# huggingface/tokenizers

Measured on AMD Instinct MI355X. Metric: GB input text/sec (whole node), GPT-2 BPE encode_batch, higher is better.
Workload: dtype u8->u32

## Files before the change

### tokenizers_amd/csrc/capi/pipeline.cpp

```cpp

int lookup_grid(const tkamd_tokenizer* t) { return std::min(3 * t->n_cu, (int)NSQ); }

struct QueueSizes {
    uint32_t sq_cap[4], row_base[4];
    size_t total;
};
static bool rerun_wanted(tkamd_tokenizer* t, Workspace* w, int raw) {
    const int err = raw & ~NOTE_BITS;
    bool again = false;
    if (raw & NOTE_ADDED_SEEN) { t->added_spec_pause = t->added_spec_len; w->force_general = true; again = true; }
    if (raw & NOTE_NFC_SEEN) { t->nfc_spec_pause = t->nfc_spec_len; w->force_nfc = true; ++t->nfc_reruns; again = true; }
    if (err == ERR_QUEUE_FULL && t->q16_div > 1) { t->q16_div = t->q16_div > 2 ? 2 : 1; again = true; }
    return again;
}

QueueSizes queue_sizes(size_t N, uint32_t q16_div, int grid) {
    QueueSizes z{};
    const size_t n_tiles = N / LOOKUP_TILE_BYTES + 1;
    const size_t per_sq = ((n_tiles + grid - 1) / grid) * LOOKUP_TILE_BYTES;
    z.sq_cap[0] = (uint32_t)(per_sq / q16_div + 64);
    z.sq_cap[1] = (uint32_t)(per_sq / 17 + 16);
    z.sq_cap[2] = (uint32_t)(per_sq / 33 + 16);
    z.sq_cap[3] = (uint32_t)(per_sq / 65 + 16);
    size_t acc = 0;
    for (int c = 0; c < 4; ++c) { z.row_base[c] = (uint32_t)acc; acc += (size_t)z.sq_cap[c] * (size_t)grid; }
    z.total = acc;
    return z;
}

void reserve_workspace(tkamd_tokenizer* t, Workspace* w, int64_t n_bytes, int64_t n_docs, uint32_t flags, bool want_meta) {
    int64_t W = (n_bytes >> 6) + 2;
    size_t N = (size_t)n_bytes;
    w->w_docmask.reserve(W * 8);
    w->w_startmask.reserve(W * 8);
    w->w_wprefix.reserve(W * 4);
    w->w_bsum.reserve((W / 256 + 2) * 4);
    w->w_tok0.reserve((N + 4) * 4);
    w->w_tmp_ids.reserve((N + 4) * 4);
    const QueueSizes z = queue_sizes(N, t->q16_div, lookup_grid(t));
    w->w_rows.reserve(z.total * 16);
    w->w_queues.reserve(z.total * 8);
    w->w_cstate.reserve((N / COMPACT_CHUNK + 4) * 8 + 16);
    w->w_chunk_lo.reserve((N / COMPACT_CHUNK + 4) * 4);
    w->w_qcount.reserve((size_t)QCNT_WORDS * 4);
    w->w_pt_tokoff.reserve((N + 4) * 4);
    w->w_ids.reserve((N + 4) * 4);
    w->w_doc_pt.reserve((n_docs + 2) * 4);
    w->w_tok_offsets.reserve((n_docs + 2) * 8);
    w->w_scalars.reserve(SC_SLOTS * 8);
    if (want_meta) w->w_pt_start.reserve((N + 4) * 4);
    if (flags & TKAMD_OFFSETS_MASK) {
        w->w_tmp_end.reserve((N + 4) * 4);
        w->w_offsets.reserve((N + 4) * 8);
    }
    if (flags & TKAMD_WANT_WORD_IDS) w->w_word_ids.reserve((N + 4) * 4);
}

using ull = unsigned long long;
enum class Step { Done, Again };

struct Batch {
    tkamd_tokenizer* t; Workspace* w; const uint8_t* d_text; const int64_t* d_doc_off; int64_t n_docs, n_bytes; const int64_t* d_seq_off; int64_t n_seqs;
    uint32_t flags; hipStream_t st; tkamd_device_result* out; const int64_t* d_inp_off; int64_t n_inputs;
    HostModel& hm = t->hm;
    Prof pf{t, w, st};
    bool mixed = false, want_words = false, want_meta = false, add_special = false, prefix_space = false, metaspace = false, words_in = false, pairs = false;
    bool typed_single = false, has_epilogue = false, want_overflow = false;
    bool precomp = false;
    int64_t n_p = 0;
    const uint8_t* p_text = nullptr; const int64_t *p_doc_off = nullptr, *d_plen = nullptr; const uint32_t* p_norig = nullptr;
    bool nfc_general = false;
    uint32_t off_mode = 0, mcap = 0;
    int64_t n_x = 0, e_n = 0, W0 = 0, W = 0;
    int64_t *sc = nullptr, *d_npretok = nullptr, *d_ntok_total = nullptr, *d_xlen = nullptr, *d_nseg = nullptr;
    uint32_t *d_counters = nullptr, *n_match = nullptr;
    int *d_err = nullptr, grid = 0;
    size_t claim_slots = 0;
    bool use_claims = false, lean = false;
    const int64_t *raw_doc_off = nullptr, *e_tok_off = nullptr;
    bool have_raw = false, have_norm = false, have_added = false;
    const ull* matchmask = nullptr;
    size_t seg_cap = 0, WX = 0;
    const uint8_t* x_text = nullptr;
    const int64_t *x_doc_off = nullptr, *x_len_dev = nullptr, *piece_off = nullptr, *piece_n_dev = nullptr;
    const uint32_t *norig = nullptr, *norig_e = nullptr;
    int64_t n_in = 0;
    bool lead_done = false;
    bool has_end = false;
    bool meta_masks = false;
    uint32_t *mlist = nullptr, *tmp_end = nullptr, *pt_end = nullptr;
    const uint32_t* pt_word = nullptr;
    WordCache wc{nullptr, nullptr, nullptr, 0u, nullptr};

    void check_request(); void zero_batch_state(); void validate_inputs(); void empty_batch();
    void build_x_text(); void pretokenize(); void run_model(); void compact_and_meta(); Step epilogue();
// ... 38 lines not shown
            while (p > 0 && !t->nfc_spec_pause.compare_exchange_weak(p, p - 1)) {}
            nfc_general = p > 0;
        }
    }
    precomp = hm.norm == NORM_PRECOMPILED;
    n_p = precomp ? (int64_t)hm.pc_growth * n_bytes + 64 : n_bytes;
    if (precomp && n_p >= (int64_t)0x55555500ll) throw Invalid("batch larger than 4 GiB behind the normalizer's bound: split it (byte offsets are 32-bit on the device)");
    n_x = (hm.norm == NORM_BERT || nfc_general) ? 3 * n_bytes + 64
          : metaspace ? 3 * n_p + 3 * (n_docs + 2 * (int64_t)mcap + 1) + 64
          : n_bytes + (prefix_space ? n_docs + (int64_t)mcap : 0);
    if (n_x >= (int64_t)0xFFFFFF00ll) throw Invalid("batch larger than 4 GiB: split it (byte offsets are 32-bit on the device)");
    const bool bpe_path = hm.model == MODEL_BPE && !hm.char_bpe && (hm.pretok == PT_BYTELEVEL_GPT2 || hm.pretok == PT_LLAMA3 || hm.pretok == PT_SPLIT_CHAIN || hm.pretok == PT_DIGITS_GPT2 ||
                                                                      hm.pretok == PT_BYTELEVEL_NOREGEX);
    const bool local_pretok = hm.pretok == PT_WHITESPACE || hm.pretok == PT_WHITESPACE_SPLIT || hm.pretok == PT_BERT;
    const bool word_models = (hm.model == MODEL_WORDLEVEL || hm.model == MODEL_WORDPIECE) && local_pretok;
    const bool char_bpe = hm.model == MODEL_BPE && hm.char_bpe && (local_pretok || metaspace);
    const bool unigram = hm.model == MODEL_UNIGRAM && metaspace;
    if (!bpe_path && !word_models && !char_bpe && !unigram)
        throw Unsupported("this build covers {ByteLevel(GPT-2 regex), Llama-3 Split+ByteLevel, ByteLevel(no regex)}+BPE and "
                          "{Whitespace,WhitespaceSplit,BertPreTokenizer}+{WordLevel,WordPiece,BPE over characters} and the U+2581 front+{BPE over characters, Unigram}");
    if (prefix_space && hm.norm != NORM_NONE) throw Unsupported("ByteLevel add_prefix_space behind a normalizer");
    words_in = n_seqs >= 0;
    if (words_in && !d_seq_off) throw Invalid("null sequence offsets");
    e_n = words_in ? n_seqs : n_docs;
    pairs = (flags & TKAMD_PAIRS) != 0 || mixed;
    if (pairs && !mixed && (e_n & 1)) throw Invalid("TKAMD_PAIRS: an odd number of documents");
    if (pairs && (flags & TKAMD_ADD_SPECIAL) && !hm.pp_pair_unsupported.empty()) throw Unsupported("add_special_tokens on a pair: " + hm.pp_pair_unsupported);
    typed_single = !pairs && hm.pp_single_typed;
    has_epilogue = hm.trunc_on || hm.pad_on || pairs || typed_single;
    want_overflow = (flags & TKAMD_WANT_OVERFLOW) != 0 && hm.trunc_on;
    W0 = (n_bytes >> 6) + 1;
    W = (n_x >> 6) + 1;
    grid = t->n_cu * 8;
}

void Batch::zero_batch_state() {
    reserve_workspace(t, w, (hm.norm == NORM_NFC && w->device_bound) ? 3 * n_bytes + 64 : n_x, n_docs, flags, want_meta);
    sc = w->w_scalars.as<int64_t>();
    d_npretok = sc + SC_NPRETOK;
    d_ntok_total = sc + SC_NTOK;
    d_xlen = sc + SC_NKEPT;
    d_err = (int*)(sc + SC_ERR);
    d_counters = (uint32_t*)(sc + SC_COUNTERS);
    const char* const claims_hook = test_hook("TKAMD_CLAIMS");
    const bool claims_on = !(claims_hook && !strcmp(claims_hook, "0"));
    use_claims = claims_on && !t->word_cache &&
                 (hm.model == MODEL_BPE || hm.model == MODEL_UNIGRAM || (hm.model == MODEL_WORDPIECE && hm.max_input_chars >= (uint32_t)WORD_MAX_KEY));
    if (use_claims) {
        int p = t->claims_pause.load();
        while (p > 0 && !t->claims_pause.compare_exchange_weak(p, p - 1)) {}
        if (p > 0) use_claims = false;
    }
    w->last_used_claims = use_claims;
    const size_t cstate_bytes = (((size_t)n_x / (size_t)COMPACT_CHUNK + 4) * 8 + 15) & ~(size_t)15;
    ZeroRegions z{};
    z.add(sc, SC_SLOTS * 8);
    if (!(hm.norm == NORM_BERT || metaspace)) z.add(w->w_docmask.p, (size_t)(W + 1) * 8);
    z.add(w->w_qcount.p, (size_t)QCNT_WORDS * 4);
    z.add(w->w_cstate.p, cstate_bytes);
    if (hm.pretok == PT_LLAMA3 && split_rule_fast(hm.split_rule)) {
        w->w_l3_tiles.reserve(l3_tileflag_words(n_x) * 8);
        z.add(w->w_l3_tiles.p, l3_tileflag_words(n_x) * 8);
    }
    if (use_claims) {
        constexpr size_t per_slot = 64;
        int bits = 18;
        while (bits < 24 && ((size_t)1 << bits) < (size_t)n_bytes / per_slot) ++bits;
        claim_slots = (size_t)1 << bits;
        w->w_claims.reserve(claim_slots * 16);
        w->w_claim_rows.reserve(claim_slots * 16);
        z.add(w->w_claims.p, claim_slots * 16);
    }
    launch_zero_regions(st, t->n_cu * 4, z);
    out->d_ids = w->w_ids.as<uint32_t>();
    out->d_tok_offsets = w->w_tok_offsets.as<int64_t>();
    out->d_n_tokens = d_ntok_total;
    out->d_n_pretokens = d_npretok;
    out->ids_capacity = ((hm.norm == NORM_NFC && w->device_bound) ? 3 * n_bytes + 64 : n_x) + 4;
    out->d_offsets = out->d_word_ids = out->d_pad_counts = out->d_enc_docs = out->d_enc_parts = nullptr;
    out->d_type_ids = out->d_seq_ids = nullptr;
    out->d_n_encodings = nullptr;
    w->cur_trim1 = nullptr;
    w->last_n_enc = -1;
    w->last_n_docs = n_docs;
    w->last_seq_off = d_seq_off;
    w->last_n_seqs = n_seqs;
    w->last_inp_off = d_inp_off;
    w->last_n_inputs = n_inputs;
}

void Batch::validate_inputs() {
    w->w_doc_off.reserve((size_t)(n_docs + 2) * 8);
    lean = n_bytes > 0 && hm.at[0].size() == 0 && hm.at[1].size() == 0 && (hm.norm == NORM_NONE || (hm.norm == NORM_NFC && !nfc_general)) && !prefix_space &&
           (hm.pretok == PT_BYTELEVEL_GPT2 || hm.pretok == PT_BYTELEVEL_NOREGEX);
    raw_doc_off = d_doc_off;
    if (!lean) {
        pf.begin("validate_csr");
        launch_validate_csr(st, d_doc_off, n_docs, n_bytes, d_err, w->w_doc_off.as<int64_t>());
        pf.end();
    }
    d_doc_off = w->w_doc_off.as<int64_t>();
    if (words_in) {
        w->w_seq_off.reserve((size_t)(n_seqs + 2) * 8);
        w->w_seq_tok_off.reserve((size_t)(n_seqs + 2) * 8);
        launch_validate_csr(st, d_seq_off, n_seqs, n_docs, d_err, w->w_seq_off.as<int64_t>());
        d_seq_off = w->w_seq_off.as<int64_t>();
        out->d_tok_offsets = w->w_seq_tok_off.as<int64_t>();
// ... 763 lines not shown
```

### tokenizers_amd/csrc/kernels.hpp

```cpp
#pragma once
#include <hip/hip_runtime_api.h>
#include <cstdint>

#include "nfc_core.hpp"
#include "precompiled_core.hpp"
#include "tables.hpp"

namespace tkamd {

struct DevTables {
    const uint16_t* uc1;
    const uint8_t* uc2;
    const uint32_t* byte_id;
    const MergeSlot* merges;
    const uint16_t* merge_disp;
    uint32_t merge_mask, merge_seed, merge_bmask;
    uint32_t newid_affine, newid_base;
    const uint32_t* char_id;
    uint32_t cb;
    int* err;
    uint32_t* probes;
    void* pub_rows;
    uint32_t* pub_pos;
    uint32_t pub_mask;
// ... 323 lines not shown
void launch_pair_lens(hipStream_t st, const PairArgs& a);
void launch_pair_overflow_scan(hipStream_t st, const PairArgs& a, int64_t* n_enc);
void launch_pair_ranges(hipStream_t st, const PairArgs& a);
void launch_pair_finalize(hipStream_t st, int grid, const PairArgs& a);
void launch_added_match(hipStream_t st, const AddedArgs& a, const uint8_t* text, int64_t n_bytes, const int64_t* len_dev, const int64_t* seg_off, int64_t n_segs,
                        const int64_t* n_segs_dev, const unsigned long long* skipmask, const uint16_t* uc1, const uint8_t* uc2, unsigned long long* candmask,
                        uint32_t* sents, uint32_t* n_sents, uint32_t* match_list, uint32_t* n_match, uint32_t cap, uint32_t len_flag, int* err);
void launch_added_detect(hipStream_t st, const AddedArgs& a, const uint8_t* text, int64_t n_bytes, const int64_t* len_dev, int* note);
void launch_scatter_matches(hipStream_t st, const uint32_t* list, const uint32_t* n_list, int64_t n_bytes, const int64_t* len_dev, unsigned long long* matchmask,
                            unsigned long long* spanmask, unsigned long long* stopmask, unsigned long long* hardmask, uint32_t* tmp_end, uint32_t* dirty);
void launch_mask_or2(hipStream_t st, unsigned long long* dst, const unsigned long long* a, const unsigned long long* b, int64_t n_words);
void launch_emit_boundaries(hipStream_t st, const unsigned long long* mask, const uint32_t* wprefix, int64_t n_bytes, const int64_t* len_dev, const int64_t* total, int64_t* out);
void launch_metaspace(hipStream_t st, const uint8_t* text, int64_t n_bytes, const int64_t* doc_off, int64_t n_docs, const unsigned long long* pstart,
                      const unsigned long long* dstart, const unsigned long long* mmask, const unsigned long long* smask, uint32_t prepend, uint8_t* olen,
                      uint32_t* wsum, uint32_t* bsum, uint32_t* wbase, int64_t* x_len, uint8_t* xtext, uint32_t* nos, int64_t* xdoc_off,
                      const int64_t* len_dev = nullptr, const uint32_t* map = nullptr);
void launch_precompiled(hipStream_t st, const PcTables& pt, const uint8_t* text, int64_t n_bytes, const int64_t* doc_off, int64_t n_docs, const unsigned long long* verbatim,
                        const unsigned long long* bound, uint8_t* olen, uint16_t* ltot, uint32_t* wsum, uint32_t* bsum, uint32_t* wbase, int64_t* x_len, uint8_t* ntext,
                        uint32_t* nos, int64_t* ndoc_off, int* err, int grid, int64_t out_cap);
void launch_pc_translate_matches(hipStream_t st, uint32_t* list, const uint32_t* n_list, const uint8_t* olen, const uint16_t* ltot, const uint32_t* wbase, int64_t n_bytes,
                                 const int64_t* x_len);
void launch_ms_units(hipStream_t st, const uint8_t* xtext, int64_t n_x, const int64_t* x_len, const unsigned long long* pmask, unsigned long long* startmask,
                     int64_t n_words, bool split);
void launch_ms_piece_rank(hipStream_t st, const unsigned long long* startmask, const uint32_t* wprefix, const unsigned long long* pmask, const uint32_t* pprefix,
                          int64_t n_x, const int64_t* x_len, uint32_t* pt_word);
void launch_translate_matches_norm(hipStream_t st, uint32_t* list, const uint32_t* n_list, const uint8_t* olen, const uint32_t* wbase, int64_t n_bytes, const int64_t* x_len);
void launch_translate_matches_prefix(hipStream_t st, uint32_t* list, const uint32_t* n_list, const unsigned long long* bmask, const uint32_t* wprefix, int64_t n_bytes,
                                     const int64_t* len_dev, const int64_t* total, const int64_t* xseg_off);
void launch_prefix_doc_csr(hipStream_t st, const int64_t* doc_off, int64_t n_docs, const unsigned long long* bmask, const uint32_t* wprefix, int64_t n_bytes,
                           const int64_t* len_dev, const int64_t* total, const int64_t* xseg_off, int64_t* xdoc_off);
void launch_mask_or(hipStream_t st, unsigned long long* dst, const unsigned long long* src, int64_t n_words, const uint32_t* n_list);
void launch_apply_matches(hipStream_t st, unsigned long long* startmask, unsigned long long* endmask, const unsigned long long* matchmask,
                          const unsigned long long* spanmask, const unsigned long long* stopmask, int64_t n_words, const uint32_t* n_list);
void launch_apply_match_ids(hipStream_t st, const uint32_t* match_list, const uint32_t* n_match, const unsigned long long* startmask,
                            const uint32_t* wprefix, uint32_t* tok0);
void launch_decode(hipStream_t st, const uint32_t* ids, const int64_t* tok_off, int64_t n_docs, int64_t n_tok, const void* entry, uint32_t n_ids,
                   const uint8_t* blob, uint32_t skip_special, uint32_t* firstmask, uint32_t* len, uint32_t* bsum, uint32_t* pos, int64_t* total,
                   int64_t* out_off, uint8_t* out_bytes_or_null, uint32_t from_end = 0, uint32_t* badmask = nullptr, uint32_t* dupmask = nullptr);
int prepare_long_kernel();
void launch_bpe_merge_long(hipStream_t st, int grid, const DevTables& t, const uint8_t* text, const QView& v, void* rows,
                           uint32_t* tmp_ids, uint32_t* tmp_end, uint32_t* list_huge, uint32_t* n_huge,
                           uint32_t* scratch, unsigned long long scratch_words, unsigned long long* scratch_used, int* err);
void launch_bpe_merge_long_only(hipStream_t st, int grid, const DevTables& t, const uint8_t* text, const QView& v, void* rows, uint32_t* tmp_ids, uint32_t* tmp_end,
                                uint32_t* list_huge, uint32_t* n_huge);
void launch_word_cache_insert(hipStream_t st, int grid, const DevTables& t, const uint8_t* text, const QView& v, const void* rows, const WordCache& wc);
void launch_compact(hipStream_t st, int grid, const uint32_t* tok0, const void* rows, const void* cache_rows, const uint32_t* tmp_ids, const int64_t* n_pretok,
                    unsigned long long* state, int64_t* n_tok, uint32_t* pt_tokoff, uint32_t* ids, const uint32_t* chunk_lo, const uint32_t* doc_pt,
                    int64_t n_docs, int64_t* tok_offsets, void* phases = nullptr, uint8_t* tok_b8 = nullptr);
int compact_grid(int n_cu);
void launch_zero_regions(hipStream_t st, int grid, const ZeroRegions& z);
void launch_zero_tail(hipStream_t st, uint8_t* p, const int64_t* len_dev, int n, unsigned long long* mask = nullptr, int64_t mask_words = 0, int grid = 1);
constexpr int CP_ITEMS_PER_LANE = 4;
constexpr int COMPACT_CHUNK = 256 * CP_ITEMS_PER_LANE;
const char* test_hook(const char* name);

}
```

### tokenizers_amd/csrc/kernels/output.hip

```cpp

constexpr int CP_NT = 256;
template <int CP_ITEMS> struct CpShape {
    static constexpr int CHUNK = CP_NT * CP_ITEMS;
    static constexpr int STAGE = CP_ITEMS * 640;
    static_assert(CP_ITEMS == 2 || CP_ITEMS == 4 || CP_ITEMS == 8, "shapes the launcher knows");
};

template <int CP_ITEMS> struct CpRows {
    uint4 row[CP_ITEMS];
    uint32_t cnt[CP_ITEMS];
};
template <int CP_ITEMS> struct CpTok0 { uint32_t w[CP_ITEMS]; };
template <int CP_ITEMS>
__device__ __forceinline__ void cp_load_tok0(const uint32_t* __restrict__ tok0, int64_t p0, int64_t P, CpTok0<CP_ITEMS>& f) {
    static_assert(CP_ITEMS == 2 || CP_ITEMS == 4 || CP_ITEMS == 8, "one 8-byte, one or two 16-byte loads of tok0 per lane");
    uint32_t* const first = f.w;
    const bool whole = p0 + CP_ITEMS <= P;
    const int64_t pl = whole ? p0 : 0;
    if (CP_ITEMS == 2) {
        const uint2 a = load_nt((const uint2*)(tok0 + pl));
        first[0] = a.x; first[CP_ITEMS - 1] = a.y;
    } else {
        const uint4 a = load_nt((const uint4*)(tok0 + pl));
        first[0] = a.x; first[1] = a.y; first[CP_ITEMS > 2 ? 2 : 0] = a.z; first[CP_ITEMS > 3 ? 3 : 0] = a.w;
// ... 30 lines not shown
    }
    return v;
}
template <int CP_ITEMS>
__device__ __forceinline__ uint32_t cp_load_rows(const CpTok0<CP_ITEMS>& f, const uint4* __restrict__ rows, const uint4* __restrict__ crows, CpRows<CP_ITEMS>& r) {
    CpGather<CP_ITEMS> g;
    cp_issue_rows<CP_ITEMS>(f, rows, crows, g);
    return cp_settle_rows<CP_ITEMS>(f, g, r);
}
template <int CP_ITEMS>
__device__ __forceinline__ uint32_t cp_load(const uint32_t* __restrict__ tok0, const uint4* __restrict__ rows, const uint4* __restrict__ crows, int64_t p0, int64_t P, CpRows<CP_ITEMS>& r) {
    CpTok0<CP_ITEMS> f;
    cp_load_tok0<CP_ITEMS>(tok0, p0, P, f);
    return cp_load_rows<CP_ITEMS>(f, rows, crows, r);
}
#define TKAMD_CP_SCATTER(DST, R, O, RAW, B8)                                                                  \
    _Pragma("unroll") for (int k = 0; k < CP_ITEMS; ++k) {                                                    \
        const uint32_t c = (R).cnt[k];                                                                        \
        if (c) {                                                                                              \
            const bool more = ((R).row[k].x >> ROW_CNT_SHIFT) == ROW_CNT_MORE;                                \
            const uint32_t keep_ = (RAW) ? 0xFFFFFFFFu : TOK_ID_MASK;                                         \
            (DST)[(O)] = ((R).row[k].x & ROW_ID_MASK) | ((RAW) && (B8) ? B8_FIRST << ROW_B8_SHIFT : 0u);      \
            if (!(RAW) && (B8)) (B8)[(O)] = (uint8_t)B8_FIRST;                                                \
            if (!more) {                                                                                      \
                if (c > 1) { (DST)[(O) + 1] = (R).row[k].y & keep_; if (!(RAW) && (B8)) (B8)[(O) + 1] = (uint8_t)((R).row[k].y >> ROW_B8_SHIFT); } \
                if (c > 2) { (DST)[(O) + 2] = (R).row[k].z & keep_; if (!(RAW) && (B8)) (B8)[(O) + 2] = (uint8_t)((R).row[k].z >> ROW_B8_SHIFT); } \
                if (c > 3) { (DST)[(O) + 3] = (R).row[k].w & keep_; if (!(RAW) && (B8)) (B8)[(O) + 3] = (uint8_t)((R).row[k].w >> ROW_B8_SHIFT); } \
            } else {                                                                                          \
                if (!(RAW) && (B8)) for (uint32_t j = 1; j < c; ++j) (B8)[(O) + j] = 0;                       \
                 \
                 \
                const uint32_t* const src_ = tmp_ids + (R).row[k].y;                                          \
                for (uint32_t j = 1; j < c; j += 4) {                                                         \
                    const Unaligned16 v_ = *(const Unaligned16*)(src_ + j);                                   \
                    (DST)[(O) + j] = v_.a;                                                                    \
                    if (j + 1 < c) (DST)[(O) + j + 1] = v_.b;                                                 \
                    if (j + 2 < c) (DST)[(O) + j + 2] = v_.c;                                                 \
                    if (j + 3 < c) (DST)[(O) + j + 3] = v_.d;                                                 \
                }                                                                                             \
            }                                                                                                 \
        }                                                                                                     \
        (O) += c;                                                                                             \
    }

template <int CP_ITEMS, bool PROF = false, bool EARLY = true>
__global__ __launch_bounds__(CP_NT, CP_ITEMS == 8 ? 2 : 5) void k_compact(const uint32_t* __restrict__ tok0, const uint4* __restrict__ rows, const uint4* __restrict__ crows,
                                                   const uint32_t* __restrict__ tmp_ids, const int64_t* __restrict__ n_pretok,
                                                   unsigned long long* __restrict__ state,
                                                   int64_t* __restrict__ n_tok, uint32_t* __restrict__ pt_tokoff, uint32_t* __restrict__ ids,
                                                   const uint32_t* __restrict__ chunk_lo, const uint32_t* __restrict__ doc_pt, int64_t n_docs,
                                                   int64_t* __restrict__ tok_offsets, unsigned long long* __restrict__ phases, uint32_t patience,
                                                   uint8_t* __restrict__ tok_b8) {
    constexpr int CP_CHUNK = CpShape<CP_ITEMS>::CHUNK, CP_STAGE = CpShape<CP_ITEMS>::STAGE;
    unsigned long long ph_t = 0ull, ph_t0 = 0ull, ph_acc[4] = {0ull, 0ull, 0ull, 0ull};
    auto tick = [&](int k) {
        if (PROF && threadIdx.x == 0) { const unsigned long long now = __builtin_amdgcn_s_memtime(); ph_acc[k] += now - ph_t; ph_t = now; }
    };
    if (PROF && threadIdx.x == 0) ph_t = ph_t0 = __builtin_amdgcn_s_memtime();
    __shared__ uint32_t sm[4];
    __shared__ uint32_t s_dlo[2], s_dhi[2];
    __shared__ uint32_t s_docpt[2][CP_NT];
    __shared__ uint32_t s_stage[2][CP_STAGE];
    __shared__ uint32_t s_loc[2][CP_CHUNK];
    __shared__ uint32_t s_tot[2];
    __shared__ unsigned long long s_lbw;
    const int64_t P = uniform_i64(*n_pretok);
    const int64_t n_chunks = (P + CP_CHUNK - 1) / CP_CHUNK;
    const int tid = (int)threadIdx.x;
    if (n_chunks == 0) {
        if (blockIdx.x == 0)
            for (int64_t d = tid; d <= n_docs; d += CP_NT) tok_offsets[d] = 0;
        return;
    }
    auto front = [&](int64_t ch, int b, const CpAhead<CP_ITEMS>& a) {
        const uint32_t dlo = a.dlo, dhi = a.dhi;
        CpRows<CP_ITEMS> r;
        const bool has_doc = dlo + (uint32_t)tid < dhi;
        uint32_t my_docpt = 0u;
        const uint32_t v = cp_load_rows<CP_ITEMS>(a.f, rows, crows, r);
        if (has_doc) my_docpt = doc_pt[dlo + (uint32_t)tid];
        uint32_t tot;
        const uint32_t ex = block256_excl_scan(v, sm, &tot);
        if (tid == 0) { lb_publish(state, ch, (unsigned long long)tot); s_tot[b] = tot; }
        if (has_doc) s_docpt[b][tid] = my_docpt;
        if (tid == 0) { s_dlo[b] = dlo; s_dhi[b] = dhi; }
        tick(0);
        uint32_t acc = ex;
#pragma unroll
        for (int k = 0; k < CP_ITEMS; ++k) { s_loc[b][tid * CP_ITEMS + k] = acc; acc += r.cnt[k]; }
        if (tot <= (uint32_t)CP_STAGE) {
            uint32_t o = ex;
            uint32_t* const dst = s_stage[b];
            TKAMD_CP_SCATTER(dst, r, o, true, tok_b8)
        }
        tick(1);
    };
    auto chunk_total = [&](int64_t hc) -> unsigned long long {
        uint32_t v = 0;
#pragma unroll 1
        for (int j = 0; j < CP_NT / 64; ++j) {
            CpRows<CP_ITEMS> r;
            v += cp_load<CP_ITEMS>(tok0, rows, crows, hc * CP_CHUNK + (int64_t)(j * 64 + (tid & 63)) * CP_ITEMS, P, r);
        }
#pragma unroll
        for (int d = 32; d >= 1; d >>= 1) v += (uint32_t)__shfl_xor((int)v, d, 64);
        return (unsigned long long)v;
    };
    auto ahead_of = [&](int64_t c, CpAhead<CP_ITEMS>& a) {
        a.dlo = a.dhi = 0u;
        if (c < n_chunks) {
            cp_load_tok0<CP_ITEMS>(tok0, c * CP_CHUNK + (int64_t)tid * CP_ITEMS, P, a.f);
            a.dlo = chunk_lo[c];
            a.dhi = c == n_chunks - 1 ? (uint32_t)n_docs + 1u : chunk_lo[c + 1];
        } else {
#pragma unroll
            for (int k = 0; k < CP_ITEMS; ++k) a.f.w[k] = 0u;
        }
    };
    int b = 0;
    CpAhead<CP_ITEMS> aa;
    {
        CpAhead<CP_ITEMS> a0;
        ahead_of(blockIdx.x, a0);
        ahead_of((int64_t)blockIdx.x + gridDim.x, aa);
        if ((int64_t)blockIdx.x < n_chunks) front(blockIdx.x, 0, a0);
    }
    for (int64_t ch = blockIdx.x; ch < n_chunks; ch += gridDim.x, b ^= 1) {
        const int64_t nxt = ch + gridDim.x;
        LbPre pre;
        CpAhead<CP_ITEMS> an;
        ahead_of(nxt + gridDim.x, an);
        if (EARLY && tid < 64) lb_prefetch(state, ch, pre);
        if (nxt < n_chunks) front(nxt, b ^ 1, aa);
        else __syncthreads();
        aa = an;
        const uint32_t tot = s_tot[b];
        if (tid < 64) {
            const unsigned long long r = EARLY ? lb_resolve_pre(state, ch, (unsigned long long)tot, patience, chunk_total, pre)
                                               : lb_resolve(state, ch, (unsigned long long)tot, patience, chunk_total);
            if (tid == 0) s_lbw = r;
        }
        __syncthreads();
        const unsigned long long base = s_lbw;
        tick(2);
        if (ch == n_chunks - 1 && tid == 0) *n_tok = (int64_t)(base + tot);
        const int64_t pc = ch * CP_CHUNK;
        if (pt_tokoff) {
#pragma unroll
            for (int i = 0; i < CP_ITEMS; ++i) {
                const int q = i * CP_NT + tid;
                if (pc + q < P) pt_tokoff[pc + q] = (uint32_t)base + s_loc[b][q];
            }
        }
        {
            const uint32_t dlo = s_dlo[b], dhi = s_dhi[b];
            for (uint32_t d = dlo + (uint32_t)tid; d < dhi; d += CP_NT) {
                uint32_t dp = s_docpt[b][(d - dlo) & (uint32_t)(CP_NT - 1)];
                if (d - dlo >= (uint32_t)CP_NT) dp = *(const volatile uint32_t*)(doc_pt + d);
                const uint32_t local = dp - (uint32_t)pc;
                tok_offsets[d] = (int64_t)(base + (local < (uint32_t)CP_CHUNK ? s_loc[b][local] : tot));
            }
        }
        if (tot <= (uint32_t)CP_STAGE) {
            if (tok_b8) {
                for (uint32_t i = (uint32_t)tid; i < tot; i += CP_NT) {
                    const uint32_t w = s_stage[b][i];
                    store_nt(ids + base + i, w & TOK_ID_MASK);
                    tok_b8[base + i] = (uint8_t)(w >> ROW_B8_SHIFT);
                }
            } else {
                for (uint32_t i = (uint32_t)tid; i < tot; i += CP_NT) store_nt(ids + base + i, s_stage[b][i]);
            }
        } else {
            const int64_t p0 = ch * CP_CHUNK + (int64_t)tid * CP_ITEMS;
            CpRows<CP_ITEMS> r;
            cp_load<CP_ITEMS>(tok0, rows, crows, p0, P, r);
            uint32_t o = s_loc[b][tid * CP_ITEMS];
            uint32_t* const dst = ids + base;
            uint8_t* const b8 = tok_b8 ? tok_b8 + base : nullptr;
            TKAMD_CP_SCATTER(dst, r, o, false, b8)
        }
        __syncthreads();
        tick(3);
    }
    if (PROF && tid == 0 && phases) {
        unsigned long long* const o = phases + (size_t)blockIdx.x * 8;
        for (int k = 0; k < 4; ++k) o[k] += ph_acc[k];
        o[7] += ph_t - ph_t0;
    }
}
#undef TKAMD_CP_SCATTER

__global__ void k_seq_tok_offsets(const int64_t* __restrict__ seq_off, int64_t n_seqs, const int64_t* __restrict__ word_tok_off,
                                  int64_t* __restrict__ seq_tok_off) {
    const int64_t s = (int64_t)blockIdx.x * blockDim.x + threadIdx.x;
    if (s <= n_seqs) seq_tok_off[s] = word_tok_off[seq_off[s]];
}
__global__ void k_word_index(const int64_t* __restrict__ seq_off, int64_t n_seqs, int64_t n_words, uint32_t* __restrict__ widx,
                             const int64_t* __restrict__ seq_tok_off, int64_t* __restrict__ first_tok) {
    const int64_t w = (int64_t)blockIdx.x * blockDim.x + threadIdx.x;
    if (w >= n_words) return;
    int64_t lo = 0, hi = n_seqs;
    while (hi - lo > 1) { const int64_t mid = (lo + hi) >> 1; if (seq_off[mid] <= w) lo = mid; else hi = mid; }
    if (widx) widx[w] = (uint32_t)(w - seq_off[lo]);
    if (first_tok) first_tok[w] = seq_tok_off[lo];
}

__device__ __forceinline__ uint32_t lead_rank(const unsigned long long* __restrict__ leadmask, const uint32_t* __restrict__ lprefix, uint32_t pos) {
    unsigned long long m = leadmask[pos >> 6];
    uint32_t b = pos & 63u;
    return lprefix[pos >> 6] + (uint32_t)__popcll(m & ((1ull << b) - 1ull));
}

__global__ __launch_bounds__(256) void k_leadmask(const uint8_t* __restrict__ text, int64_t n_bytes, unsigned long long* __restrict__ leadmask) {
    const int64_t q = (int64_t)blockIdx.x * 256 + threadIdx.x;
    const int64_t i = q * 16;
    uint32_t bits = 0u;
    if (i < n_bytes) {
        const uint4 v = *(const uint4*)(text + i);
        auto four = [](uint32_t w) -> uint32_t {
            const uint32_t cont = (w >> 7) & (~w >> 6) & 0x01010101u;
            return (((cont ^ 0x01010101u) * 0x01020408u) >> 24) & 0xFu;
        };
        bits = four(v.x) | (four(v.y) << 4) | (four(v.z) << 8) | (four(v.w) << 12);
        const int64_t left = n_bytes - i;
        if (left < 16) bits &= (1u << left) - 1u;
    }
    unsigned long long m = (unsigned long long)bits << (16 * (threadIdx.x & 3));
    m |= __shfl_xor(m, 1, 64);
    m |= __shfl_xor(m, 2, 64);
    if ((threadIdx.x & 3) == 0 && i <= n_bytes) leadmask[i >> 6] = m;
}

__device__ __forceinline__ uint32_t norig_end(const MetaArgs& a, uint32_t k) {
    if (a.norig_e) return a.norig_e[k];
    const uint32_t i = a.norig[k], b = a.text[i];
    return i + (b < 0xC0u ? 1u : b < 0xE0u ? 2u : b < 0xF0u ? 3u : 4u);
}

__device__ __forceinline__ void meta_one_token(const MetaArgs& a, int64_t p, int64_t d, uint32_t s, uint32_t e, bool is_match, uint32_t o, uint32_t j,
                                               uint32_t rel, uint32_t rel_end, uint32_t xdoc, uint32_t odoc, uint32_t word,
// ... 402 lines not shown
```

### tokenizers_amd/csrc/kernels/results.hip

```cpp

constexpr uint32_t TOK_ROW = 0x80000000u;
constexpr uint32_t TOK_ONE = 0x40000000u;
constexpr uint32_t TOK_ID_MASK = 0x00FFFFFFu;
constexpr uint32_t TOK_SLOT = TOK_ROW | TOK_ONE, TOK_REF_MASK = 0x3FFFFFFFu;
constexpr uint32_t ROW_CNT_SHIFT = 28, ROW_CNT_MORE = 15u, ROW_ID_MASK = 0x0FFFFFFFu;
constexpr uint32_t ROW_WHOLE_WORD = 0xFFFFFFFFu;

struct __attribute__((aligned(8))) QItem { uint32_t s, len; };
constexpr uint32_t QLEN_CLAIM = 0x80000000u;
__device__ __forceinline__ uint32_t qitem_len(uint32_t len_word) { return len_word & ~QLEN_CLAIM; }

__device__ __forceinline__ uint32_t qview_prefix(const QView& v, uint32_t* s_pre) {
    constexpr int PER = NSQ / 64;
    static_assert(NSQ % 64 == 0, "sub-queues per lane");
    __syncthreads();
    if (threadIdx.x < 64) {
        uint32_t c[PER], sum = 0;
#pragma unroll
        for (int k = 0; k < PER; ++k) { c[k] = min(v.counts[(threadIdx.x * PER + k) * QCNT_STRIDE], v.sq_cap); sum += c[k]; }
        uint32_t run = wave_incl_scan(sum) - sum;
#pragma unroll
        for (int k = 0; k < PER; ++k) { run += c[k]; s_pre[threadIdx.x * PER + k + 1] = run; }
        if (threadIdx.x == 0) s_pre[0] = 0u;
    }
    __syncthreads();
    return s_pre[NSQ];
}
__device__ __forceinline__ uint32_t qview_pos(const uint32_t* s_pre, uint32_t sq_cap, uint32_t item) {
    uint32_t lo = 0, hi = NSQ;
#pragma unroll
    for (int it = 0; it < 10; ++it) {
        static_assert(NSQ <= 1024, "binary search depth");
        const uint32_t mid = (lo + hi) >> 1;
        if (hi - lo > 1) { if (s_pre[mid] <= item) lo = mid; else hi = mid; }
    }
    return lo * sq_cap + (item - s_pre[lo]);
}

__device__ __forceinline__ uint32_t row_count(const uint4& row) {
    const uint32_t cf = row.x >> ROW_CNT_SHIFT;
    return cf < ROW_CNT_MORE ? cf : row.z;
}
constexpr uint32_t ROW_B8_SHIFT = 24;
constexpr uint32_t B8_FIRST = 0xE0u;
__device__ __forceinline__ uint32_t row_boundary(const uint8_t* __restrict__ text, uint32_t s, uint32_t pos, bool snap) {
    uint32_t code = 0u;
    if (snap && (text[s + pos] & 0xC0u) == 0x80u) {
        uint32_t back = 1u, fwd = 1u;
        while (back < 3u && (text[s + pos - back] & 0xC0u) == 0x80u) ++back;
        while (fwd < 3u && (text[s + pos + fwd] & 0xC0u) == 0x80u) ++fwd;
        code = back == 1u ? (fwd == 1u ? 1u : fwd == 2u ? 2u : 4u) : back == 2u ? (fwd == 1u ? 3u : 5u) : 6u;
    }
    return (pos | (code << 5)) << ROW_B8_SHIFT;
}
__device__ __forceinline__ uint32_t b8_back(uint32_t v) { return (0x3994u >> ((v >> 5) * 2u)) & 3u; }
__device__ __forceinline__ uint32_t b8_fwd(uint32_t v) { return (0x1B64u >> ((v >> 5) * 2u)) & 3u; }

__device__ __forceinline__ uint4 make_row(uint32_t count, uint32_t s, uint32_t id0, uint32_t id1, uint32_t id2, uint32_t id3) {
    return count <= 4u ? make_uint4(id0 | (count << ROW_CNT_SHIFT), id1, id2, id3) : make_uint4(id0 | (ROW_CNT_MORE << ROW_CNT_SHIFT), s, count, 0u);
}

constexpr unsigned long long LB_AGG = 1ull << 62, LB_PREFIX = 2ull << 62, LB_FLAGS = 3ull << 62, LB_VALUE = ~LB_FLAGS;

__device__ __forceinline__ void lb_store(unsigned long long* p, unsigned long long v) {
    __hip_atomic_store(p, v, __ATOMIC_RELAXED, __HIP_MEMORY_SCOPE_AGENT);
}
__device__ __forceinline__ unsigned long long lb_load(const unsigned long long* p) {
    return __hip_atomic_load(p, __ATOMIC_RELAXED, __HIP_MEMORY_SCOPE_AGENT);
}
__device__ __forceinline__ void lb_publish(unsigned long long* __restrict__ state, int64_t ch, unsigned long long total) {
    lb_store(&state[ch], (ch == 0 ? LB_PREFIX : LB_AGG) | total);
}
constexpr uint32_t LB_PATIENCE = 1024;
template <class Help>
__device__ __forceinline__ unsigned long long lb_resolve_from(unsigned long long* __restrict__ state, int64_t ch, int64_t i, unsigned long long run, unsigned long long total,
                                                              uint32_t patience, Help&& help) {
    const int lane = lane_id();
    uint32_t polls = 0u;
    while (true) {
        const int64_t idx = i - lane;
        unsigned long long st;
        uint64_t empty, pref;
        do {
            st = idx >= 0 ? lb_load(&state[idx]) : LB_PREFIX;
            empty = __ballot((st & LB_FLAGS) == 0ull);
            pref = __ballot((st & LB_FLAGS) == LB_PREFIX);
            if (pref) {
                const int first = __ffsll((unsigned long long)pref) - 1;
                empty &= (first >= 63) ? ~0ull : ((2ull << first) - 1ull);
            }
            if (empty && ++polls > patience) {
                int k = (int)((blockIdx.x + polls) % (uint32_t)__popcll((unsigned long long)empty));
                uint64_t e = empty;
                for (; k > 0; --k) e &= e - 1ull;
                const int64_t hc = i - (int64_t)(__ffsll((unsigned long long)e) - 1);
                const unsigned long long t = help(hc);
                if (lane == 0) atomicCAS(&state[hc], 0ull, (hc == 0 ? LB_PREFIX : LB_AGG) | t);
                patience = 8u;
                polls = 0u;
            }
        } while (empty);
        const int first = pref ? __ffsll((unsigned long long)pref) - 1 : 63;
        unsigned long long v = (lane <= first) ? (st & LB_VALUE) : 0ull;
#pragma unroll
        for (int d = 32; d >= 1; d >>= 1) v += __shfl_xor(v, d, 64);
        run += v;
        if (pref) break;
        i -= 64;
    }
    if (lane == 0) lb_store(&state[ch], LB_PREFIX | (run + total));
    return run;
}
template <class Help>
__device__ __forceinline__ unsigned long long lb_resolve(unsigned long long* __restrict__ state, int64_t ch, unsigned long long total, uint32_t patience, Help&& help) {
    if (ch == 0) return 0ull;
    return lb_resolve_from(state, ch, ch - 1, 0ull, total, patience, help);
}

constexpr int LB_PRE_W = 2;
struct LbPre { unsigned long long st[LB_PRE_W]; };
__device__ __forceinline__ void lb_prefetch(const unsigned long long* __restrict__ state, int64_t ch, LbPre& p) {
    const int lane = lane_id();
#pragma unroll
    for (int r = 0; r < LB_PRE_W; ++r) {
        const int64_t idx = ch - 1 - 64 * r - lane;
        p.st[r] = idx >= 0 ? lb_load(&state[idx]) : LB_PREFIX;
    }
}
template <class Help>
__device__ __forceinline__ unsigned long long lb_resolve_pre(unsigned long long* __restrict__ state, int64_t ch, unsigned long long total, uint32_t patience, Help&& help,
                                                             const LbPre& p) {
    const int lane = lane_id();
    if (ch == 0) return 0ull;
    unsigned long long acc = 0ull;
    bool done = false;
    int used = 0;
#pragma unroll
    for (int r = 0; r < LB_PRE_W; ++r) {
        if (!done && used == r) {
            const unsigned long long st = p.st[r];
            uint64_t empty = __ballot((st & LB_FLAGS) == 0ull);
            const uint64_t pref = __ballot((st & LB_FLAGS) == LB_PREFIX);
            const int first = pref ? __ffsll((unsigned long long)pref) - 1 : 63;
            if (pref) empty &= (first >= 63) ? ~0ull : ((2ull << first) - 1ull);
            if (!empty) {
                acc += (lane <= first) ? (st & LB_VALUE) : 0ull;
                used = r + 1;
                done = pref != 0ull;
            }
        }
    }
    unsigned long long run = acc;
#pragma unroll
    for (int d = 32; d >= 1; d >>= 1) run += __shfl_xor(run, d, 64);
    if (done) {
        if (lane == 0) lb_store(&state[ch], LB_PREFIX | (run + total));
        return run;
    }
    return lb_resolve_from(state, ch, ch - 1 - 64 * (int64_t)used, run, total, patience, help);
}
```

Baseline: 272.9.

## Replace decoupled look-back with per-block carry plus grouped chunk aggregates

The compact kernel's cross-chunk prefix scan no longer uses a decoupled look-back chain with inclusive-prefix flags. Each block now carries its own running total from its previous chunk and sums only the chunks published in between. Whole 64-chunk groups are read through atomically accumulated group words that pack a count and a sum, so only partial edge groups need per-chunk loads. This is meant to shorten the serial look-back latency. In exchange every publish does an extra atomicAdd and the workspace needs extra group words. The profiling accumulators are also moved into shared memory.

```diff
diff --git a/tokenizers_amd/csrc/capi/pipeline.cpp b/tokenizers_amd/csrc/capi/pipeline.cpp
--- a/tokenizers_amd/csrc/capi/pipeline.cpp
+++ b/tokenizers_amd/csrc/capi/pipeline.cpp
@@ -40,7 +40,7 @@
     const QueueSizes z = queue_sizes(N, t->q16_div, lookup_grid(t));
     w->w_rows.reserve(z.total * 16);
     w->w_queues.reserve(z.total * 8);
-    w->w_cstate.reserve((N / COMPACT_CHUNK + 4) * 8 + 16);
+    w->w_cstate.reserve(lb_state_words(N / COMPACT_CHUNK + 4) * 8 + 16);
     w->w_chunk_lo.reserve((N / COMPACT_CHUNK + 4) * 4);
     w->w_qcount.reserve((size_t)QCNT_WORDS * 4);
     w->w_pt_tokoff.reserve((N + 4) * 4);
@@ -185,7 +185,7 @@
         if (p > 0) use_claims = false;
     }
     w->last_used_claims = use_claims;
-    const size_t cstate_bytes = (((size_t)n_x / (size_t)COMPACT_CHUNK + 4) * 8 + 15) & ~(size_t)15;
+    const size_t cstate_bytes = (lb_state_words((size_t)n_x / (size_t)COMPACT_CHUNK + 4) * 8 + 15) & ~(size_t)15;
     ZeroRegions z{};
     z.add(sc, SC_SLOTS * 8);
     if (!(hm.norm == NORM_BERT || metaspace)) z.add(w->w_docmask.p, (size_t)(W + 1) * 8);
diff --git a/tokenizers_amd/csrc/kernels.hpp b/tokenizers_amd/csrc/kernels.hpp
--- a/tokenizers_amd/csrc/kernels.hpp
+++ b/tokenizers_amd/csrc/kernels.hpp
@@ -399,6 +399,9 @@
 void launch_zero_tail(hipStream_t st, uint8_t* p, const int64_t* len_dev, int n, unsigned long long* mask = nullptr, int64_t mask_words = 0, int grid = 1);
 constexpr int CP_ITEMS_PER_LANE = 4;
 constexpr int COMPACT_CHUNK = 256 * CP_ITEMS_PER_LANE;
+constexpr int LB_GROUP_CHUNKS = 64, LB_GROUP_STRIDE = 32;
+constexpr size_t lb_group_base(size_t n_chunks) { return (n_chunks + 15) & ~(size_t)15; }
+constexpr size_t lb_state_words(size_t max_chunks) { return lb_group_base(max_chunks) + (max_chunks / LB_GROUP_CHUNKS + 1) * LB_GROUP_STRIDE; }
 const char* test_hook(const char* name);
 
 }
diff --git a/tokenizers_amd/csrc/kernels/output.hip b/tokenizers_amd/csrc/kernels/output.hip
--- a/tokenizers_amd/csrc/kernels/output.hip
+++ b/tokenizers_amd/csrc/kernels/output.hip
@@ -106,11 +106,15 @@
                                                    int64_t* __restrict__ tok_offsets, unsigned long long* __restrict__ phases, uint32_t patience,
                                                    uint8_t* __restrict__ tok_b8) {
     constexpr int CP_CHUNK = CpShape<CP_ITEMS>::CHUNK, CP_STAGE = CpShape<CP_ITEMS>::STAGE;
-    unsigned long long ph_t = 0ull, ph_t0 = 0ull, ph_acc[4] = {0ull, 0ull, 0ull, 0ull};
+    __shared__ unsigned long long s_ph[PROF ? 5 : 1];
+    unsigned long long ph_t = 0ull;
     auto tick = [&](int k) {
-        if (PROF && threadIdx.x == 0) { const unsigned long long now = __builtin_amdgcn_s_memtime(); ph_acc[k] += now - ph_t; ph_t = now; }
+        if (PROF && threadIdx.x == 0) { const unsigned long long now = __builtin_amdgcn_s_memtime(); s_ph[k] += now - ph_t; ph_t = now; }
     };
-    if (PROF && threadIdx.x == 0) ph_t = ph_t0 = __builtin_amdgcn_s_memtime();
+    if (PROF && threadIdx.x == 0) {
+        for (int k = 0; k < 4; ++k) s_ph[k] = 0ull;
+        s_ph[4] = ph_t = __builtin_amdgcn_s_memtime();
+    }
     __shared__ uint32_t sm[4];
     __shared__ uint32_t s_dlo[2], s_dhi[2];
     __shared__ uint32_t s_docpt[2][CP_NT];
@@ -121,6 +125,7 @@
     const int64_t P = uniform_i64(*n_pretok);
     const int64_t n_chunks = (P + CP_CHUNK - 1) / CP_CHUNK;
     const int tid = (int)threadIdx.x;
+    unsigned long long* const groups = lb_groups(state, n_chunks);
     if (n_chunks == 0) {
         if (blockIdx.x == 0)
             for (int64_t d = tid; d <= n_docs; d += CP_NT) tok_offsets[d] = 0;
@@ -135,7 +140,7 @@
         if (has_doc) my_docpt = doc_pt[dlo + (uint32_t)tid];
         uint32_t tot;
         const uint32_t ex = block256_excl_scan(v, sm, &tot);
-        if (tid == 0) { lb_publish(state, ch, (unsigned long long)tot); s_tot[b] = tot; }
+        if (tid == 0) { lb_publish(state, groups, ch, (unsigned long long)tot); s_tot[b] = tot; }
         if (has_doc) s_docpt[b][tid] = my_docpt;
         if (tid == 0) { s_dlo[b] = dlo; s_dhi[b] = dhi; }
         tick(0);
@@ -179,23 +184,26 @@
         ahead_of((int64_t)blockIdx.x + gridDim.x, aa);
         if ((int64_t)blockIdx.x < n_chunks) front(blockIdx.x, 0, a0);
     }
+    unsigned long long carry = 0ull;
     for (int64_t ch = blockIdx.x; ch < n_chunks; ch += gridDim.x, b ^= 1) {
         const int64_t nxt = ch + gridDim.x;
+        const int64_t prev = ch == (int64_t)blockIdx.x ? -1 : ch - (int64_t)gridDim.x;
         LbPre pre;
         CpAhead<CP_ITEMS> an;
         ahead_of(nxt + gridDim.x, an);
-        if (EARLY && tid < 64) lb_prefetch(state, ch, pre);
+        if (EARLY && tid < 64) lb_prefetch(state, groups, prev, ch, pre);
         if (nxt < n_chunks) front(nxt, b ^ 1, aa);
         else __syncthreads();
         aa = an;
         const uint32_t tot = s_tot[b];
         if (tid < 64) {
-            const unsigned long long r = EARLY ? lb_resolve_pre(state, ch, (unsigned long long)tot, patience, chunk_total, pre)
-                                               : lb_resolve(state, ch, (unsigned long long)tot, patience, chunk_total);
+            if (!EARLY) lb_prefetch(state, groups, prev, ch, pre);
+            const unsigned long long r = carry + lb_resolve(state, groups, prev, ch, patience, chunk_total, pre);
             if (tid == 0) s_lbw = r;
         }
         __syncthreads();
         const unsigned long long base = s_lbw;
+        carry = (unsigned long long)uniform_i64((int64_t)(base + tot));
         tick(2);
         if (ch == n_chunks - 1 && tid == 0) *n_tok = (int64_t)(base + tot);
         const int64_t pc = ch * CP_CHUNK;
@@ -239,8 +247,8 @@
     }
     if (PROF && tid == 0 && phases) {
         unsigned long long* const o = phases + (size_t)blockIdx.x * 8;
-        for (int k = 0; k < 4; ++k) o[k] += ph_acc[k];
-        o[7] += ph_t - ph_t0;
+        for (int k = 0; k < 4; ++k) o[k] += s_ph[k];
+        o[7] += ph_t - s_ph[4];
     }
 }
 #undef TKAMD_CP_SCATTER
diff --git a/tokenizers_amd/csrc/kernels/results.hip b/tokenizers_amd/csrc/kernels/results.hip
--- a/tokenizers_amd/csrc/kernels/results.hip
+++ b/tokenizers_amd/csrc/kernels/results.hip
@@ -60,7 +60,10 @@
     return count <= 4u ? make_uint4(id0 | (count << ROW_CNT_SHIFT), id1, id2, id3) : make_uint4(id0 | (ROW_CNT_MORE << ROW_CNT_SHIFT), s, count, 0u);
 }
 
-constexpr unsigned long long LB_AGG = 1ull << 62, LB_PREFIX = 2ull << 62, LB_FLAGS = 3ull << 62, LB_VALUE = ~LB_FLAGS;
+constexpr unsigned long long LB_AGG = 1ull << 62, LB_VALUE = LB_AGG - 1ull;
+constexpr int LB_GCOUNT_SHIFT = 56;
+constexpr unsigned long long LB_GSUM = (1ull << LB_GCOUNT_SHIFT) - 1ull;
+static_assert(LB_GROUP_CHUNKS == 64, "one wavefront-wide load reads a group's states");
 
 __device__ __forceinline__ void lb_store(unsigned long long* p, unsigned long long v) {
     __hip_atomic_store(p, v, __ATOMIC_RELAXED, __HIP_MEMORY_SCOPE_AGENT);
@@ -68,94 +71,75 @@
 __device__ __forceinline__ unsigned long long lb_load(const unsigned long long* p) {
     return __hip_atomic_load(p, __ATOMIC_RELAXED, __HIP_MEMORY_SCOPE_AGENT);
 }
-__device__ __forceinline__ void lb_publish(unsigned long long* __restrict__ state, int64_t ch, unsigned long long total) {
-    lb_store(&state[ch], (ch == 0 ? LB_PREFIX : LB_AGG) | total);
+__device__ __forceinline__ unsigned long long* lb_groups(unsigned long long* state, int64_t n_chunks) { return state + lb_group_base((size_t)n_chunks); }
+__device__ __forceinline__ unsigned long long* lb_group_word(unsigned long long* groups, int64_t g) { return groups + g * LB_GROUP_STRIDE; }
+__device__ __forceinline__ void lb_publish(unsigned long long* __restrict__ state, unsigned long long* __restrict__ groups, int64_t ch, unsigned long long total) {
+    lb_store(&state[ch], LB_AGG | total);
+    atomicAdd(lb_group_word(groups, ch / LB_GROUP_CHUNKS), (1ull << LB_GCOUNT_SHIFT) | total);
 }
 constexpr uint32_t LB_PATIENCE = 1024;
+
+struct LbCut { int64_t lo, fe, gl, gh, hi; };
+__device__ __forceinline__ LbCut lb_cut(int64_t prev, int64_t ch) {
+    LbCut c;
+    c.lo = prev + 1;
+    c.hi = ch;
+    c.gl = (c.lo + LB_GROUP_CHUNKS - 1) / LB_GROUP_CHUNKS;
+    c.gh = max(ch / LB_GROUP_CHUNKS, c.gl);
+    c.fe = min(c.gl * LB_GROUP_CHUNKS, ch);
+    return c;
+}
+struct LbPre { unsigned long long a, g, b; };
+__device__ __forceinline__ void lb_prefetch(unsigned long long* __restrict__ state, unsigned long long* __restrict__ groups, int64_t prev, int64_t ch, LbPre& p) {
+    const int lane = lane_id();
+    const LbCut c = lb_cut(prev, ch);
+    p.a = c.lo + lane < c.fe ? lb_load(&state[c.lo + lane]) : 0ull;
+    p.g = c.gl + lane < c.gh ? lb_load(lb_group_word(groups, c.gl + lane)) : 0ull;
+    p.b = c.hi - 1 - lane >= c.gh * LB_GROUP_CHUNKS ? lb_load(&state[c.hi - 1 - lane]) : 0ull;
+}
+struct LbWait { uint32_t patience, polls; };
 template <class Help>
-__device__ __forceinline__ unsigned long long lb_resolve_from(unsigned long long* __restrict__ state, int64_t ch, int64_t i, unsigned long long run, unsigned long long total,
-                                                              uint32_t patience, Help&& help) {
+__device__ __forceinline__ unsigned long long lb_window(unsigned long long* __restrict__ state, int64_t first, int step, int n, unsigned long long st, LbWait& w, Help&& help) {
     const int lane = lane_id();
-    uint32_t polls = 0u;
-    while (true) {
-        const int64_t idx = i - lane;
-        unsigned long long st;
-        uint64_t empty, pref;
-        do {
-            st = idx >= 0 ? lb_load(&state[idx]) : LB_PREFIX;
-            empty = __ballot((st & LB_FLAGS) == 0ull);
-            pref = __ballot((st & LB_FLAGS) == LB_PREFIX);
-            if (pref) {
-                const int first = __ffsll((unsigned long long)pref) - 1;
-                empty &= (first >= 63) ? ~0ull : ((2ull << first) - 1ull);
-            }
-            if (empty && ++polls > patience) {
-                int k = (int)((blockIdx.x + polls) % (uint32_t)__popcll((unsigned long long)empty));
-                uint64_t e = empty;
-                for (; k > 0; --k) e &= e - 1ull;
-                const int64_t hc = i - (int64_t)(__ffsll((unsigned long long)e) - 1);
-                const unsigned long long t = help(hc);
-                if (lane == 0) atomicCAS(&state[hc], 0ull, (hc == 0 ? LB_PREFIX : LB_AGG) | t);
-                patience = 8u;
-                polls = 0u;
-            }
-        } while (empty);
-        const int first = pref ? __ffsll((unsigned long long)pref) - 1 : 63;
-        unsigned long long v = (lane <= first) ? (st & LB_VALUE) : 0ull;
-#pragma unroll
-        for (int d = 32; d >= 1; d >>= 1) v += __shfl_xor(v, d, 64);
-        run += v;
-        if (pref) break;
-        i -= 64;
+    const bool want = lane < n;
+    const int64_t idx = first + (int64_t)step * lane;
+    uint64_t empty;
+    while ((empty = __ballot(want && st == 0ull)) != 0ull) {
+        if (++w.polls > w.patience) {
+            int k = (int)((blockIdx.x + w.polls) % (uint32_t)__popcll((unsigned long long)empty));
+            uint64_t e = empty;
+            for (; k > 0; --k) e &= e - 1ull;
+            const int64_t hc = first + (int64_t)step * (__ffsll((unsigned long long)e) - 1);
+            const unsigned long long t = help(hc);
+            if (lane == 0) atomicCAS(&state[hc], 0ull, LB_AGG | t);
+            w.patience = 8u;
+            w.polls = 0u;
+        }
+        if (want && st == 0ull) st = lb_load(&state[idx]);
     }
-    if (lane == 0) lb_store(&state[ch], LB_PREFIX | (run + total));
-    return run;
+    return want ? (st & LB_VALUE) : 0ull;
 }
 template <class Help>
-__device__ __forceinline__ unsigned long long lb_resolve(unsigned long long* __restrict__ state, int64_t ch, unsigned long long total, uint32_t patience, Help&& help) {
-    if (ch == 0) return 0ull;
-    return lb_resolve_from(state, ch, ch - 1, 0ull, total, patience, help);
-}
-
-constexpr int LB_PRE_W = 2;
-struct LbPre { unsigned long long st[LB_PRE_W]; };
-__device__ __forceinline__ void lb_prefetch(const unsigned long long* __restrict__ state, int64_t ch, LbPre& p) {
+__device__ __forceinline__ unsigned long long lb_resolve(unsigned long long* __restrict__ state, unsigned long long* __restrict__ groups, int64_t prev, int64_t ch,
+                                                         uint32_t patience, Help&& help, const LbPre& p) {
     const int lane = lane_id();
-#pragma unroll
-    for (int r = 0; r < LB_PRE_W; ++r) {
-        const int64_t idx = ch - 1 - 64 * r - lane;
-        p.st[r] = idx >= 0 ? lb_load(&state[idx]) : LB_PREFIX;
-    }
-}
-template <class Help>
-__device__ __forceinline__ unsigned long long lb_resolve_pre(unsigned long long* __restrict__ state, int64_t ch, unsigned long long total, uint32_t patience, Help&& help,
-                                                             const LbPre& p) {
-    const int lane = lane_id();
-    if (ch == 0) return 0ull;
-    unsigned long long acc = 0ull;
-    bool done = false;
-    int used = 0;
-#pragma unroll
-    for (int r = 0; r < LB_PRE_W; ++r) {
-        if (!done && used == r) {
-            const unsigned long long st = p.st[r];
-            uint64_t empty = __ballot((st & LB_FLAGS) == 0ull);
-            const uint64_t pref = __ballot((st & LB_FLAGS) == LB_PREFIX);
-            const int first = pref ? __ffsll((unsigned long long)pref) - 1 : 63;
-            if (pref) empty &= (first >= 63) ? ~0ull : ((2ull << first) - 1ull);
-            if (!empty) {
-                acc += (lane <= first) ? (st & LB_VALUE) : 0ull;
-                used = r + 1;
-                done = pref != 0ull;
-            }
+    const LbCut c = lb_cut(prev, ch);
+    LbWait w{patience, 0u};
+    unsigned long long acc = lb_window(state, c.lo, 1, (int)(c.fe - c.lo), p.a, w, help);
+    acc += lb_window(state, c.hi - 1, -1, (int)(c.hi - c.gh * LB_GROUP_CHUNKS), p.b, w, help);
+    for (int64_t g0 = c.gl; g0 < c.gh; g0 += 64) {
+        const bool want = g0 + lane < c.gh;
+        unsigned long long gw = g0 == c.gl ? p.g : 0ull;
+        if (want && (gw >> LB_GCOUNT_SHIFT) != (unsigned long long)LB_GROUP_CHUNKS) gw = lb_load(lb_group_word(groups, g0 + lane));
+        const bool whole = (gw >> LB_GCOUNT_SHIFT) == (unsigned long long)LB_GROUP_CHUNKS;
+        acc += want && whole ? (gw & LB_GSUM) : 0ull;
+        for (uint64_t m = __ballot(want && !whole); m; m &= m - 1ull) {
+            const int64_t gx = g0 + (__ffsll((unsigned long long)m) - 1);
+            const unsigned long long st = lb_load(&state[gx * LB_GROUP_CHUNKS + lane]);
+            acc += lb_window(state, gx * LB_GROUP_CHUNKS, 1, LB_GROUP_CHUNKS, st, w, help);
         }
     }
-    unsigned long long run = acc;
 #pragma unroll
-    for (int d = 32; d >= 1; d >>= 1) run += __shfl_xor(run, d, 64);
-    if (done) {
-        if (lane == 0) lb_store(&state[ch], LB_PREFIX | (run + total));
-        return run;
-    }
-    return lb_resolve_from(state, ch, ch - 1 - 64 * (int64_t)used, run, total, patience, help);
+    for (int d = 32; d >= 1; d >>= 1) acc += __shfl_xor(acc, d, 64);
+    return acc;
 }
```

After: 284.8, median of 6. +4.3%, better.
